# balisujohn/tortoise.cpp

Measured on AMD Instinct MI355X. Metric: audio-seconds/sec end-to-end (AR+diffusion+vocoder), 16 cands x 80 steps, higher is better.
Workload: dtype f16 MFMA inputs / f32 accumulate (diffusion, vocoder convs); f32 weights, f16 KV (AR)

## Files before the change

tortoise.cpp_amd/csrc/api.cpp:

```cpp
#include "common.h"
#include <sched.h>
#include <cctype>
#include <cstddef>
#include <cmath>
#include <algorithm>
#include <chrono>
#include <fstream>
#include <new>

using namespace tts;

hipEvent_t tts::prof_event(tts_ctx *c) {
  if (!c->ev_pool.empty()) { hipEvent_t e = c->ev_pool.back(); c->ev_pool.pop_back(); return e; }
  hipEvent_t e = nullptr;
  (void)hipEventCreate(&e);
  return e;
}

template <class F>
static int guarded(tts_ctx *c, F body) {
  try {
    return body();
  } catch (const std::bad_alloc &) {
    return fail(c, TTS_ERR_LIMIT, "out of host memory");
// ... 139 lines not shown
}

int tts_set_option(tts_ctx *c, const char *key, double value) {
  if (!c || !key) return TTS_ERR_ARG;
  std::string k(key);
  if (k == "gn_eps") c->gn_eps = (float)value;
  else if (k == "ggml_lut") c->ggml_lut = value != 0;
  else if (k.rfind("prof_only:", 0) == 0) {
    if (value != 0) c->prof_filter.push_back(k.substr(10));
    else c->prof_filter.clear();
  }
  else if (k == "device_topk") c->device_topk = value != 0;
  else if (k == "sampler_threads") {
    if (c->sampler_pool) { sampler_pool_free(c->sampler_pool); c->sampler_pool = nullptr; }
    c->sampler_threads = value < 0 ? -1 : (int)value;
  }
  else if (k == "share_uncond") c->share_uncond = value != 0;
  else if (k == "prof_stride") c->prof_stride = value < 1 ? 1 : (int)value;
  else if (k == "diff_graph") c->diff_graph = value != 0;
  else if (k == "dec_f32_mfma") c->dec_f32_mfma = value != 0;
  else if (k == "attn_f32") c->attn_f32 = value != 0;
  else if (k == "attn_proj_f16") c->attn_proj_f16 = value != 0;
  else if (k == "proj_dual_b") c->proj_dual_b = value != 0;
  else if (k == "gemm_wreg") c->gemm_wreg = value == 1 ? tts_ctx::GEMM_WREG_ALL : value == 2 ? 1 : value == 3 ? 2 : value == 4 ? 4 : 0;
  else if (k == "lc_attn_f32") c->lc_attn_f32 = value != 0;
  else if (k == "latency_mode") c->latency_mode = value != 0;
  else if (k == "fp16_check") c->fp16_check = value != 0;
  else if (k == "rng_fast_normal") c->rng_fast_normal = value != 0;
  else if (k == "noise_pipeline") c->noise_pipeline = value != 0;
  else if (k == "load_device_pack") c->load_device_pack = value != 0;
  else if (k == "load_threads") c->load_threads = value < 0 ? 0 : value > 64 ? 64 : (int)value;
  else if (k == "attn_q64") c->attn_q64 = value < 0 ? 0 : value > 2 ? 2 : (int)value;
  else if (k == "hoist_integrator") c->hoist_integrator = value < 0 ? 0 : (int)value;
  else if (k == "attn_f32_drop") c->attn_f32_drop = (int)value & 7;
  else if (k == "ar_weights") {
    if (value != 0 && value != 1 && value != 2) return fail(c, TTS_ERR_ARG, "ar_weights: 0 (f32), 1 (fp16) or 2 (fp8 e4m3)");
    c->ar_weights = (int)value;
  }
  else if (k == "diff_sampler") {
    if (const char *e = diff_control_error(0, value)) return fail(c, TTS_ERR_ARG, "%s", e);
    c->diff_sampler = (int)value;
  }
  else if (k == "ddim_eta") {
    if (const char *e = diff_control_error(1, value)) return fail(c, TTS_ERR_ARG, "%s", e);
    c->ddim_eta = value;
  }
  else if (k == "cond_free_k") {
// ... 712 lines not shown
```

tortoise.cpp_amd/csrc/common.h:

```cpp
#pragma once
#include "../../include/tortoise_mi355x.h"
#include <hip/hip_runtime.h>
#include <cstdarg>
#include <cstdint>
#include <cstdio>
#include <cstring>
#include <functional>
#include <map>
#include <memory>
#include <random>
#include <algorithm>
#include <atomic>
#include <condition_variable>
#include <mutex>
#include <new>
#include <string>
#include <thread>
#include <vector>

namespace tts {

struct HostTensor {
  std::vector<float> data;
  int64_t ne[4] = {1, 1, 1, 1};
// ... 98 lines not shown
  tts::DiffCondEncState *dcond = nullptr;
  tts::HifiganState *hifigan = nullptr;
  tts::AfeState *afe = nullptr;
  tts::Tokenizer *tok = nullptr;
  tts::ArSession *session = nullptr;
  tts::DiffSession *diff_session = nullptr;
  tts::SamplerPool *sampler_pool = nullptr;
  tts::SamplerParams ar_sp;
  int ar_penalty_scope = 0;
  int device_topk = 1;
  int time_mlp_retries = 0;
  int topk_fallbacks = 0;
  int sampler_threads = -1;
  bool share_uncond = true;
  int rng_shard_offset = 0, rng_shard_total = 0;
  std::vector<int32_t> stop_schedule;
  std::vector<int32_t> ar_stopped;
  bool prof_on = false;
  std::vector<std::string> prof_filter;
  int prof_stride = 1;
  int ar_weights = 0;
  int dec_f32_mfma = 0;
  int attn_f32 = 0;
  static constexpr int GEMM_WREG_ALL = 7;
  int gemm_wreg = GEMM_WREG_ALL;
  int proj_dual_b = 1;
  int attn_f32_drop = 0;
  int lc_attn_f32 = 1;
  int attn_proj_f16 = 0;
  int fp16_check = 0;
  int64_t fp16_bad_weights[2] = {0, 0};
  void *fp16_counts = nullptr;
  int rng_fast_normal = 1;
  int noise_pipeline = 1;
  int load_device_pack = 1;
  int load_threads = 0;
  int attn_q64 = 0;
  int hoist_integrator = 1;
  int latency_mode = 0;
  int diff_sampler = 0;
  double ddim_eta = 0;
  float cond_free_k = 2.0f;
  int cond_free = 1;
  double diff_temperature = 1.0;
  int last_diff_rows = -1, last_diff_seqs = 0;
  bool capturing = false;
  int stream_recaptures = 0;
// ... 324 lines not shown
```

tortoise.cpp_amd/csrc/diffusion.hip:

```cpp
#include "common.h"
#include "gemm_f16.h"
#include <algorithm>
#include <chrono>
#include <cmath>

namespace tts {

static constexpr int C = 1024, NHEAD = 16, XTC = 128 ;
static constexpr int LAT_MAX_ROWS = 2048;
static constexpr int HOIST_MAX_ROWS = 16384;

__device__ __forceinline__ float silu_dev(float x, int lut) {
  if (lut == 1) {
    float xr = __half2float(__float2half_rn(x));
    return __half2float(__float2half_rn(xr / (1.0f + expf(-xr))));
  }
  if (lut == 2) return x / (1.0f + expf(-x));
  return x * __builtin_amdgcn_rcpf(1.0f + __builtin_amdgcn_exp2f(x * -1.44269504088896f));
}

__global__ __launch_bounds__(256) void gn_stats_kernel(const float *__restrict__ x, const int *__restrict__ seq_start,
                                                       const int *__restrict__ seq_len, float eps, float2 *__restrict__ stats) {
  __shared__ float sh[8];
  const int grp = blockIdx.x, s = blockIdx.y, T = seq_len[s];
// ... 738 lines not shown
}

__global__ void philox_fill_kernel(float *__restrict__ x, int64_t n, uint64_t seed, uint32_t stream, uint32_t step) {
  int64_t i = (int64_t)blockIdx.x * blockDim.x + threadIdx.x;
  if (i < n) x[i] = philox_normal(seed, stream, step, (uint32_t)i);
}
__global__ void scale_xT_kernel(float *__restrict__ x, int64_t n, float temperature) {
  int64_t i = (int64_t)blockIdx.x * blockDim.x + threadIdx.x;
  if (i < n) x[i] = temperature * x[i];
}

__global__ void rows_to_ct_kernel(const float *__restrict__ net, int row0, int T, int nch, int ld, float *__restrict__ out) {
  int i = blockIdx.x * blockDim.x + threadIdx.x;
  if (i < nch * T) {
    int ch = i / T, t = i - ch * T;
    out[i] = net[(size_t)(row0 + t) * ld + ch];
  }
}

struct AttnDev {
  float *norm_g, *norm_b, *qkv_b, *proj_b, *bias_tab;
  __half *qkv_w, *proj_w;
  __half *qkv_wf;
  __half *proj_w_split;
  float proj_alpha;
};
struct ResDev { float *in_g, *in_b, *in_bias, *emb_w, *emb_b, *out_g, *out_b, *out_bias; __half *in_w, *out_w, *in_wf, *out_wf; };

struct Layout {
  int ns = 0, rows = 0;
  std::vector<int> start, len;
  DevBuf d_row_seq, d_row_t, d_start, d_len, d_chunk_seq;
  int build(tts_ctx *ctx, const std::vector<int> &lens) {
    has_seq_step = false; ss_step_stride = 0; gn_parts.clear();
    ns = (int)lens.size();
    len = lens;
    start.resize(ns);
    int r = 8;
    for (int s = 0; s < ns; s++) { start[s] = r; r = (r + lens[s] + 1 + 7) & ~7; }
    rows = (r + 127) & ~127;
    std::vector<int> rs(rows, -1), rt(rows, 0);
    for (int s = 0; s < ns; s++)
      for (int t = 0; t < lens[s]; t++) { rs[start[s] + t] = s; rt[start[s] + t] = t; }
    TTS_HIP(ctx, d_row_seq.reserve(rows * 4)); TTS_HIP(ctx, d_row_t.reserve(rows * 4));
    TTS_HIP(ctx, d_start.reserve(ns * 4)); TTS_HIP(ctx, d_len.reserve(ns * 4));
    TTS_HIP(ctx, hipMemcpy(d_row_seq.p, rs.data(), rows * 4, hipMemcpyHostToDevice));
// ... 229 lines not shown
  int f32(const std::string &name, int64_t n, float **dst) {
    const HostTensor *t = get(name, n);
    if (!t) return TTS_ERR_FORMAT;
    return put(t->data, dst);
  }
  int conv16(const std::string &name, int cout, int cin, int k, int cout_pad, int cin_pad, __half **dst, __half **dst_frag = nullptr) {
    const HostTensor *t = get(name, (int64_t)cout * cin * k);
    if (!t) return TTS_ERR_FORMAT;
    std::vector<__half> h((size_t)cout_pad * k * cin_pad, __float2half(0.f));
    const float *w = t->data.data();
    for (int co = 0; co < cout; co++)
      for (int ci = 0; ci < cin; ci++)
        for (int tap = 0; tap < k; tap++)
          h[(size_t)co * k * cin_pad + (size_t)tap * cin_pad + ci] = __float2half_rn(w[((size_t)co * cin + ci) * k + tap]);
    if (dst_frag) {
      std::vector<__half> f(h.size());
      for (int n = 0; n < cout_pad; n++)
        for (int tap = 0; tap < k; tap++)
          for (int c = 0; c < cin_pad; c++) f[gemm_wfrag3_index(n, tap, c, cout_pad, cin_pad)] = h[((size_t)n * k + tap) * cin_pad + c];
      if (int r = put(f, dst_frag)) return r;
    }
    return put(h, dst);
  }
  int attn(const std::string &p, AttnDev &a) {
    int r;
    if ((r = f32(p + ".norm.weight", C, &a.norm_g))) return r;
    if ((r = f32(p + ".norm.bias", C, &a.norm_b))) return r;
    if ((r = conv16(p + ".qkv.weight", 3 * C, C, 1, 3 * C, C, &a.qkv_w, &a.qkv_wf))) return r;
    if ((r = f32(p + ".qkv.bias", 3 * C, &a.qkv_b))) return r;
    if ((r = conv16(p + ".proj_out.weight", C, C, 1, C, C, &a.proj_w))) return r;
    {
      const HostTensor *t = get(p + ".proj_out.weight", (int64_t)C * C);
      std::vector<__half> sp((size_t)C * 2 * C);
      float amax = 0.f;
      for (float v : t->data) amax = std::max(amax, std::fabs(v));
      if (!std::isfinite(amax)) { fail(ctx, TTS_ERR_FORMAT, "tensor '%s.proj_out.weight' holds a non-finite value", p.c_str()); return TTS_ERR_FORMAT; }
      int e = 14;
      while (e > -14 && std::ldexp(amax, e) >= 30000.0f) e--;
      const float scale = std::ldexp(1.0f, e);
      a.proj_alpha = 1.0f / scale;
      for (int n = 0; n < C; n++)
        for (int k = 0; k < C; k++) {
          const float w = t->data[(size_t)n * C + k] * scale;
          const __half hi = __float2half_rn(w);
          sp[(size_t)n * 2 * C + k] = hi;
          sp[(size_t)n * 2 * C + C + k] = __float2half_rn(w - __half2float(hi));
        }
      long long bad[2] = {0, 0};
      for (const __half &h : sp) {
        const float v = std::fabs(__half2float(h));
        if (!(v <= 65504.0f)) bad[0]++;
        else if (v > 60000.0f) bad[1]++;
      }
      if (bad[0] | bad[1]) { std::lock_guard<std::mutex> lk(mu); ctx->fp16_bad_weights[0] += bad[0]; ctx->fp16_bad_weights[1] += bad[1]; }
      if ((r = put(sp, &a.proj_w_split))) return r;
    }
    if ((r = f32(p + ".proj_out.bias", C, &a.proj_b))) return r;
    const HostTensor *t = get(p + ".relative_pos_embeddings.relative_attention_bias.weight", 32 * 16);
    if (!t) return TTS_ERR_FORMAT;
    std::vector<float> tab(16 * 128);
    for (int h = 0; h < 16; h++)
      for (int sgn = 0; sgn < 2; sgn++)
        for (int d = 0; d < 64; d++) {
          int bucket = sgn ? rel_bucket(0, d) : rel_bucket(d, 0);
          if (d == 0) bucket = rel_bucket(0, 0);
          tab[h * 128 + sgn * 64 + d] = t->data[(size_t)bucket * 16 + h] * 8.0f;
        }
    return put(tab, &a.bias_tab);
  }
  int res(const std::string &p, ResDev &w) {
    int r;
    if ((r = f32(p + ".in_layers.0.weight", C, &w.in_g))) return r;
    if ((r = f32(p + ".in_layers.0.bias", C, &w.in_b))) return r;
    if ((r = conv16(p + ".in_layers.2.weight", C, C, 1, C, C, &w.in_w, &w.in_wf))) return r;
    if ((r = f32(p + ".in_layers.2.bias", C, &w.in_bias))) return r;
    if ((r = f32(p + ".emb_layers.1.weight", 2 * C * C, &w.emb_w))) return r;
    if ((r = f32(p + ".emb_layers.1.bias", 2 * C, &w.emb_b))) return r;
    if ((r = f32(p + ".out_layers.0.weight", C, &w.out_g))) return r;
// ... 8 lines not shown
int diff_load(tts_ctx *ctx, const char *path) {
  ctx->fp16_bad_weights[0] = ctx->fp16_bad_weights[1] = 0;
  WeightFile wf;
  std::string err;
  int rc = read_weight_file(path, wf, err);
  if (rc != TTS_OK) return fail(ctx, rc, "diffusion_model_load: %s", err.c_str());
  std::unique_ptr<DiffState> st(new DiffState());
  Loader ld{ctx, st.get(), wf, {}};
  while (wf.has("latent_conditioner." + std::to_string(st->n_lc + 1) + ".norm.weight")) st->n_lc++;
  while (wf.has("conditioning_timestep_integrator." + std::to_string(st->n_integ) + ".resblk.in_layers.0.weight")) st->n_integ++;
  while (wf.has("layers." + std::to_string(st->n_main) + ".resblk.in_layers.0.weight")) st->n_main++;
  while (wf.has("layers." + std::to_string(st->n_main + st->n_tail) + ".in_layers.0.weight")) st->n_tail++;
  st->lc_attn.resize(st->n_lc);
  st->integ_res.resize(st->n_integ); st->integ_attn.resize(st->n_integ);
  st->main_res.resize(st->n_main); st->main_attn.resize(st->n_main);
  st->tail_res.resize(st->n_tail);
  std::vector<std::function<int()>> jobs;
  DiffState *S = st.get();
#define J(x) jobs.emplace_back([&ld, S]() -> int { (void)S; return (x); })
  J(ld.f32("diffusion_conditioning_latent", 2 * C, &S->cond_latent));
  J(ld.f32("unconditioned_embedding", C, &S->uncond_emb));
  J(ld.conv16("latent_conditioner.0.weight", C, C, 3, C, C, &S->lc_w));
  J(ld.f32("latent_conditioner.0.bias", C, &S->lc_bias));
  for (int i = 0; i < st->n_lc; i++) jobs.emplace_back([&ld, S, i]() { return ld.attn("latent_conditioner." + std::to_string(i + 1), S->lc_attn[i]); });
  J(ld.f32("code_norm.weight", C, &S->code_g));
  J(ld.f32("code_norm.bias", C, &S->code_b));
  J(ld.f32("time_embed.0.weight", C * C, &S->te0_w)); J(ld.f32("time_embed.0.bias", C, &S->te0_b));
  J(ld.f32("time_embed.2.weight", C * C, &S->te2_w)); J(ld.f32("time_embed.2.bias", C, &S->te2_b));
  for (int i = 0; i < st->n_integ; i++) {
    jobs.emplace_back([&ld, S, i]() { return ld.res("conditioning_timestep_integrator." + std::to_string(i) + ".resblk", S->integ_res[i]); });
    jobs.emplace_back([&ld, S, i]() { return ld.attn("conditioning_timestep_integrator." + std::to_string(i) + ".attn", S->integ_attn[i]); });
  }
  J(ld.conv16("inp_block.weight", C, 100, 3, C, XTC, &S->inp_w));
  J(ld.f32("inp_block.bias", C, &S->inp_bias));
  J(ld.conv16("integrating_conv.weight", C, 2 * C, 1, C, 2 * C, &S->integ_w));
  J(ld.f32("integrating_conv.bias", C, &S->integ_bias));
  for (int i = 0; i < st->n_main; i++) {
    jobs.emplace_back([&ld, S, i]() { return ld.res("layers." + std::to_string(i) + ".resblk", S->main_res[i]); });
    jobs.emplace_back([&ld, S, i]() { return ld.attn("layers." + std::to_string(i) + ".attn", S->main_attn[i]); });
  }
  for (int i = 0; i < st->n_tail; i++) jobs.emplace_back([&ld, S, i]() { return ld.res("layers." + std::to_string(S->n_main + i), S->tail_res[i]); });
  J(ld.f32("out.0.weight", C, &S->outn_g)); J(ld.f32("out.0.bias", C, &S->outn_b));
  J(ld.conv16("out.2.weight", 200, C, 3, 256, C, &S->out_w));
  jobs.emplace_back([&ld, S]() -> int {
    const HostTensor *t = ld.get("out.2.bias", 200);
    if (!t) return TTS_ERR_FORMAT;
    std::vector<float> b(256, 0.f);
    std::copy(t->data.begin(), t->data.end(), b.begin());
    return ld.put(b, &S->out_bias);
  });
#undef J
  if (int r = run_parallel(ctx, (int)jobs.size(), [&](int i) { return jobs[i](); })) return r;
  for (auto &kv : wf.t)
    if (!ld.used.count(kv.first)) return fail(ctx, TTS_ERR_FORMAT, "unknown tensor '%s' in model file", kv.first.c_str());
  TTS_HIP(ctx, hipFuncSetAttribute((const void *)diff_attn_f32_kernel, hipFuncAttributeMaxDynamicSharedMemorySize, ATT32_LDS));
  if (ctx->diff) diff_free(ctx->diff);
  ctx->diff = st.release();
  return TTS_OK;
}

#define CHECK(x) do { int _r = (x); if (_r) return _r; } while (0)

// ... 349 lines not shown
        diff_attn_kernel<2, 2><<<nq * NHEAD * lay.ns, 256, att_lds<2>(), ctx->stream>>>(wk.qk16.as<__half>(), wk.vt16.as<__half>(), wk.rows + 128,
                                                                                    lay.d_start.as<int>(), lay.d_len.as<int>(), w.bias_tab, wk.ATT16(), nq);
    }
    TTS_HIP(ctx, hipGetLastError());
  }
  CHECK(fp16_check(ctx, wk.ATT16(), (size_t)lay.rows * C));
  if (f32 && (ctx->attn_f32_drop & 4)) TTS_HIP(ctx, hipMemsetAsync(wk.att16_lo.p, 0, (size_t)(wk.rows + 2) * C * 2, ctx->stream));
  DBG_SUM("attn out", wk.ATT16(), (size_t)lay.rows * C * 2);
  if (f32) {
    GemmArgs p = gemm_base(lay, wk.ATT16(), C, 3, C, w.proj_w_split, C, w.proj_b);
    p.A[0] = wk.ATT16(); p.A[1] = wk.att16_lo.as<__half>() + C; p.A[2] = wk.ATT16();
    p.row_off[0] = p.row_off[1] = p.row_off[2] = 0;
    p.custom_w = 1; p.ldw_ = 2 * C; p.w_off_[0] = 0; p.w_off_[1] = 0; p.w_off_[2] = C;
    p.mode = st_out ? GEMM_OUT_F32_SCALED_STATS : GEMM_OUT_F32_SCALED; p.alpha = w.proj_alpha; p.outF = X; p.ldo = C; p.resid = X;
    p.st_out = st_out; p.st_stripe_ll = (int)st->gn_stripe_ll; p.chunk_seq = lay.d_chunk_seq.as<int>();
    return gemm(ctx, "diff_gemm", p, lay, 0, C);
  }
  if (!ctx->attn_proj_f16) {
    GemmArgs p = gemm_base(lay, wk.ATT16(), C, 2, C, w.proj_w_split, C, w.proj_b);
    p.custom_w = 1; p.ldw_ = 2 * C; p.w_off_[0] = 0; p.w_off_[1] = C;
    p.mode = st_out ? GEMM_OUT_F32_SCALED_STATS : GEMM_OUT_F32_SCALED; p.alpha = w.proj_alpha; p.outF = X; p.ldo = C; p.resid = X;
    p.st_out = st_out; p.st_stripe_ll = (int)st->gn_stripe_ll; p.chunk_seq = lay.d_chunk_seq.as<int>();
    p.dual_b = ctx->proj_dual_b;
    CHECK(gemm(ctx, "diff_gemm", p, lay, 0, C));
    DBG_SUM("attn proj", X, (size_t)lay.rows * C * 4);
    return TTS_OK;
  }
  GemmArgs p = gemm_base(lay, wk.ATT16(), C, 1, C, w.proj_w, C, w.proj_b);
  p.mode = st_out ? GEMM_OUT_F32_STATS : GEMM_OUT_F32; p.outF = X; p.ldo = C; p.resid = X;
  p.st_out = st_out; p.st_stripe_ll = (int)st->gn_stripe_ll; p.chunk_seq = lay.d_chunk_seq.as<int>();
  CHECK(gemm(ctx, "diff_gemm", p, lay));
  DBG_SUM("attn proj", X, (size_t)lay.rows * C * 4);
  return TTS_OK;
}

static int res_block(tts_ctx *ctx, DiffState *st, const Layout &lay, Work &wk, float *X, const ResDev &w, const float *ss,
                     const float *Xin = nullptr, const float *Hpre = nullptr, const long long *st_hpre = nullptr) {
  const float *xin = Xin ? Xin : X;
  const bool lat = st->lat && (Hpre ? st_hpre != nullptr : wk.st_x != nullptr);
  const long long *st_h = st_hpre;
  if (!Hpre) {
    long long *slot = lat ? st->new_stats_slot() : nullptr;
    CHECK(res_in_layers(ctx, st, lay, wk, xin, w, wk.H(), lat ? wk.st_x : nullptr, slot));
    Hpre = wk.H();
    st_h = slot;
  }
// ... 832 lines not shown
```

tortoise.cpp_amd/csrc/gemm_f16.h:

```cpp
#pragma once
#include <hip/hip_fp16.h>
#include <hip/hip_runtime.h>
#include <algorithm>
#include <cmath>
#include <cstdlib>
#include <type_traits>

namespace tts {

typedef _Float16 half8 __attribute__((ext_vector_type(8)));
typedef float floatx4 __attribute__((ext_vector_type(4)));

enum { GEMM_OUT_F32 = 0, GEMM_OUT_F16 = 1, GEMM_OUT_QKV = 2, GEMM_OUT_QKV_SPLIT = 3, GEMM_OUT_F32_SCALED = 4, GEMM_OUT_F32_STATS = 5, GEMM_OUT_F32_SCALED_STATS = 6 };
constexpr bool gemm_mode_qkv(int mode) { return mode == GEMM_OUT_QKV || mode == GEMM_OUT_QKV_SPLIT; }
constexpr bool gemm_mode_f32(int mode) { return mode == GEMM_OUT_F32 || mode == GEMM_OUT_F32_SCALED || mode == GEMM_OUT_F32_STATS || mode == GEMM_OUT_F32_SCALED_STATS; }
constexpr bool gemm_mode_scaled(int mode) { return mode == GEMM_OUT_F32_SCALED || mode == GEMM_OUT_F32_SCALED_STATS; }
constexpr bool gemm_mode_stats(int mode) { return mode == GEMM_OUT_F32_STATS || mode == GEMM_OUT_F32_SCALED_STATS; }

struct GemmArgs {
  const __half *A[3];
  int row_off[3];
  int nseg, kseg;
  int lda;
  const __half *W;
  int ldw_, w_off_[3], custom_w;
  const __half *Wf;
  int wreg;
  int M, N;
  const float *bias;
  const int *row_seq;
  float *outF; int ldo; const float *resid;
  __half *outH; int ldh;
  __half *outVt; int ldvt;
  __half *outH2, *outVt2;
  float alpha;
  long long *st_out;
  int st_stripe_ll;
  const int *chunk_seq;
  int dual_b;
  int mode;
  int th, cn;
  int ku;
};


__device__ __forceinline__ int lds_swz(int row) { return ((row >> 1) & 3) << 1; }
__device__ __forceinline__ int lds_off(int row, int chunk) { return row * 128 + ((chunk ^ lds_swz(row)) << 4); }

typedef const void __attribute__((address_space(1))) *gptr_t;
// ... 460 lines not shown
#pragma unroll
            for (int r = 0; r < 4; r++) v[r] = gd[r] ? 0.f : acc[i][j][r] + bv[j];
            const size_t o = (size_t)(h * 64 + (w0 - 128) + j * 16 + fr) * g.ldvt + rbase;
            *(uint2 *)(g.outVt + o) = pack_half4(v[0], v[1], v[2], v[3]);
            if (MODE == GEMM_OUT_QKV_SPLIT) *(uint2 *)(g.outVt2 + o) = pack_half4(split_lo(v[0]), split_lo(v[1]), split_lo(v[2]), split_lo(v[3]));
          }
        }
      }
      return;
    }
  }
  const int col0 = c0 + fq * 4;
  float4 b4[2];
  int sq[MI];
#pragma unroll
  for (int j = 0; j < 2; j++) b4[j] = *(const float4 *)(bp + col0 + j * 16);
#pragma unroll
  for (int i = 0; i < MI; i++) sq[i] = sp[m0 + min(i, nblk - 1) * 16 + fr];
#pragma unroll
  for (int j = 0; j < 2; j++) b4[j] = hb ? b4[j] : make_float4(0.f, 0.f, 0.f, 0.f);
#pragma unroll
  for (int i = 0; i < MI; i++) sq[i] = hs ? sq[i] : 0;
  auto finish = [&](int i, int j) {
    float4 v = make_float4(acc[i][j][0] + b4[j].x, acc[i][j][1] + b4[j].y, acc[i][j][2] + b4[j].z, acc[i][j][3] + b4[j].w);
    if (sq[i] < 0) v = make_float4(0.f, 0.f, 0.f, 0.f);
    return v;
  };
  if (MODE == GEMM_OUT_F32) {
#pragma unroll
    for (int i = 0; i < MI; i++) {
      if (i < nblk) {
        float *op = g.outF + (size_t)(m0 + i * 16 + fr) * g.ldo + col0;
#pragma unroll
        for (int j = 0; j < 2; j++) *(float4 *)(op + j * 16) = finish(i, j);
      }
    }
  } else {
    const int h = c0 / 192, w0 = c0 - h * 192;
#pragma unroll
    for (int i = 0; i < MI; i++) {
      if (i < nblk) {
        __half *op = g.outH + (size_t)(m0 + i * 16 + fr) * g.ldh + h * 128 + w0 + fq * 4;
#pragma unroll
        for (int j = 0; j < 2; j++) {
          const float4 v = finish(i, j);
          *(uint2 *)(op + j * 16) = pack_half4(v.x, v.y, v.z, v.w);
          if (MODE == GEMM_OUT_QKV_SPLIT)
            *(uint2 *)(g.outH2 + (op - g.outH) + j * 16) = pack_half4(split_lo(v.x), split_lo(v.y), split_lo(v.z), split_lo(v.w));
        }
      }
    }
// ... 335 lines not shown
  issue_slab(0, 0);
  issue_w(0, 0, std::integral_constant<int, 0>{});
  for (int kc = 0; kc < nchunks; kc += 2) {
    chunk(kc, std::integral_constant<int, 0>{});
    if (kc + 1 < nchunks) chunk(kc + 1, std::integral_constant<int, 1>{});
  }
  wreg_wait<0>(w[0][0][0], w[0][0][1], w[0][1][0], w[0][1][1]);
  wreg_wait<0>(w[1][0][0], w[1][0][1], w[1][1][0], w[1][1][1]);
  gemm_epilogue_conv3_wreg<MI, RESID>(g, acc, m0, n0, nblk, wave, fr, fq);
}

template <bool RESID>
static __global__ __launch_bounds__(256, 4) void gemm_f16_conv3_wreg_kernel(GemmArgs g) {
  const int tid = threadIdx.x, lane = tid & 63, wave = __builtin_amdgcn_readfirstlane(tid >> 6);
  int m0, n0, nblk;
  if (!gemm_vh_tile(g, m0, n0, nblk)) return;
  if (nblk > 4) gemm_conv3_wreg_body<8, RESID>(g, m0, n0, nblk, lane, wave);
  else gemm_conv3_wreg_body<4, RESID>(g, m0, n0, nblk, lane, wave);
}
static inline bool gemm_takes_conv3_wreg(const GemmArgs &g, int th) {
  return g.wreg > 0 && g.Wf && gemm_is_conv3(g) && th == 8 && g.mode == GEMM_OUT_F32;
}

static inline int gemm_auto_th(int M, int N) {
  const int maxb = ((M >> 4) + 7) / 8 + 1, NT = N >> 7;
  int th = 2;
  while (th < 8 && 8 * ((maxb + th - 1) / th) * NT > 1024) th *= 2;
  return th;
}

enum { GEMM_KERNEL_VH = 0, GEMM_KERNEL_DUALB = 1, GEMM_KERNEL_CONV3 = 2, GEMM_KERNEL_WREG = 3, GEMM_KERNEL_CONV3_WREG = 4 };
struct GemmPlan {
  hipError_t err;
  int kernel;
  int th, ku, cn;
  int grid, lds;
};
static inline GemmPlan gemm_plan(const GemmArgs &g) {
  GemmPlan p = {};
  const int NT = g.N >> 7, ktot = g.nseg * g.kseg, nb = g.M >> 4;
  p.err = hipSuccess;
  if (gemm_mode_scaled(g.mode)) {
    int e;
    if (!(g.alpha != 0.f) || std::fabs(std::frexp(g.alpha, &e)) != 0.5f) p.err = hipErrorInvalidValue;
  }
  if (gemm_mode_stats(g.mode) && (!g.st_out || !g.chunk_seq || g.st_stripe_ll <= 0)) p.err = hipErrorInvalidValue;
  if (g.dual_b && !(gemm_mode_scaled(g.mode) && g.nseg == 2 && g.custom_w && g.A[0] == g.A[1] && g.row_off[0] == g.row_off[1])) p.err = hipErrorInvalidValue;
  int ku = (g.ku == 2 || g.ku == 4) && (g.kseg % (64 * g.ku)) == 0 ? g.ku : 1;
  p.cn = NT;
  if (NT > 8)
    for (p.cn = NT; p.cn > 1; p.cn--)
      if (NT % p.cn == 0 && (size_t)p.cn * 128 * ktot * 2 <= (size_t)2560 * 1024) break;
  const int maxb = (nb + 7) / 8 + 1;
  p.th = g.th > 0 ? g.th : gemm_auto_th(g.M, g.N);
  if (g.th <= 0 && g.ku == 0 && NT <= 8 && 8 * ((maxb + 3) / 4) * NT <= 256 && (g.kseg % 256) == 0) {
    p.th = 4;
    if (!gemm_is_conv3(g)) ku = g.dual_b ? 2 : 4;
  }
  int mt_max = 0;
  for (int x = 0; x < 8; x++) {
    const int b0 = (int)((long long)nb * x >> 3), b1 = (int)((long long)nb * (x + 1) >> 3);
    mt_max = std::max(mt_max, (b1 - b0 + p.th - 1) / p.th);
  }
  p.grid = 8 * mt_max * NT;
  if (gemm_takes_wreg(g, p.th, ku)) { p.kernel = GEMM_KERNEL_WREG; p.ku = 1; p.lds = GEMM_WREG_LDS; }
  else if (gemm_takes_conv3_wreg(g, p.th)) { p.kernel = GEMM_KERNEL_CONV3_WREG; p.ku = 1; p.lds = CONV3_WREG_LDS; }
  else if (gemm_is_conv3(g)) { p.kernel = GEMM_KERNEL_CONV3; p.ku = 1; p.lds = CONV3_VH_LDS; }
  else if (g.dual_b) { p.kernel = GEMM_KERNEL_DUALB; p.ku = ku == 2 ? 2 : 1; p.lds = p.ku * GEMM_DUALB_LDS; }
  else { p.kernel = GEMM_KERNEL_VH; p.ku = ku; p.lds = ku * GEMM_VH_LDS; }
  return p;
}

static_assert(GEMM_DUALB_LDS <= 48 * 1024 && GEMM_VH_LDS <= 48 * 1024 && GEMM_WREG_LDS <= 48 * 1024 && CONV3_WREG_LDS <= 48 * 1024 && CONV3_VH_LDS > 48 * 1024, "which launches raise their dynamic LDS limit");
template <void (*KERN)(GemmArgs)> static inline void gemm_launch(const GemmPlan &p, const GemmArgs &g, hipStream_t s) {
  if (p.lds > 48 * 1024) {
    static bool raised = false;
    if (!raised) { (void)hipFuncSetAttribute((const void *)KERN, hipFuncAttributeMaxDynamicSharedMemorySize, p.lds); raised = true; }
  }
  KERN<<<p.grid, 256, p.lds, s>>>(g);
}
template <int KU> static inline void gemm_launch_vh(const GemmPlan &p, const GemmArgs &g, hipStream_t s) {
  constexpr int WGS = KU == 1 ? 4 : KU == 2 ? 2 : 1;
  switch (g.mode) {
    case GEMM_OUT_F32: return gemm_launch<gemm_f16_vh_kernel<GEMM_OUT_F32, WGS, KU>>(p, g, s);
    case GEMM_OUT_F16: return gemm_launch<gemm_f16_vh_kernel<GEMM_OUT_F16, WGS, KU>>(p, g, s);
    case GEMM_OUT_QKV: return gemm_launch<gemm_f16_vh_kernel<GEMM_OUT_QKV, WGS, KU>>(p, g, s);
    case GEMM_OUT_QKV_SPLIT: return gemm_launch<gemm_f16_vh_kernel<GEMM_OUT_QKV_SPLIT, WGS, KU>>(p, g, s);
    case GEMM_OUT_F32_SCALED: return gemm_launch<gemm_f16_vh_kernel<GEMM_OUT_F32_SCALED, WGS, KU>>(p, g, s);
    case GEMM_OUT_F32_STATS: return gemm_launch<gemm_f16_vh_kernel<GEMM_OUT_F32_STATS, WGS, KU>>(p, g, s);
    default: return gemm_launch<gemm_f16_vh_kernel<GEMM_OUT_F32_SCALED_STATS, WGS, KU>>(p, g, s);
  }
}
template <int KU> static inline void gemm_launch_dualb(const GemmPlan &p, const GemmArgs &g, hipStream_t s) {
  if (g.mode == GEMM_OUT_F32_SCALED) gemm_launch<gemm_f16_vh_dualb_kernel<GEMM_OUT_F32_SCALED, KU>>(p, g, s);
  else gemm_launch<gemm_f16_vh_dualb_kernel<GEMM_OUT_F32_SCALED_STATS, KU>>(p, g, s);
}
// ... 1 lines not shown
  if (g.mode == GEMM_OUT_F32) gemm_launch<gemm_f16_conv3_vh_kernel<GEMM_OUT_F32>>(p, g, s);
  else if (g.mode == GEMM_OUT_F32_STATS) gemm_launch<gemm_f16_conv3_vh_kernel<GEMM_OUT_F32_STATS>>(p, g, s);
  else gemm_launch<gemm_f16_conv3_vh_kernel<GEMM_OUT_F16>>(p, g, s);
}
static inline void gemm_launch_conv3_wreg(const GemmPlan &p, const GemmArgs &g, hipStream_t s) {
  if (g.resid) gemm_launch<gemm_f16_conv3_wreg_kernel<true>>(p, g, s);
  else gemm_launch<gemm_f16_conv3_wreg_kernel<false>>(p, g, s);
}
static inline void gemm_launch_wreg(const GemmPlan &p, const GemmArgs &g, hipStream_t s) {
  if (g.mode == GEMM_OUT_F32) gemm_launch<gemm_f16_wreg_kernel<GEMM_OUT_F32>>(p, g, s);
  else if (g.mode == GEMM_OUT_QKV) gemm_launch<gemm_f16_wreg_kernel<GEMM_OUT_QKV>>(p, g, s);
  else gemm_launch<gemm_f16_wreg_kernel<GEMM_OUT_QKV_SPLIT>>(p, g, s);
}

static inline hipError_t launch_gemm_f16(const GemmArgs &g, hipStream_t s) {
  const GemmPlan p = gemm_plan(g);
  if (p.err != hipSuccess) return p.err;
  GemmArgs gg = g;
  gg.th = p.th;
  gg.cn = p.cn;
  if (p.kernel == GEMM_KERNEL_WREG) gemm_launch_wreg(p, gg, s);
  else if (p.kernel == GEMM_KERNEL_CONV3_WREG) gemm_launch_conv3_wreg(p, gg, s);
  else if (p.kernel == GEMM_KERNEL_CONV3) gemm_launch_conv3(p, gg, s);
  else if (p.kernel == GEMM_KERNEL_DUALB) p.ku == 2 ? gemm_launch_dualb<2>(p, gg, s) : gemm_launch_dualb<1>(p, gg, s);
  else p.ku == 4 ? gemm_launch_vh<4>(p, gg, s) : p.ku == 2 ? gemm_launch_vh<2>(p, gg, s) : gemm_launch_vh<1>(p, gg, s);
  return hipGetLastError();
}

}
```

Baseline: 137.5.

## Add register-resident weight dual-B GEMM kernel for diffusion attention projection

Adds a new dual-B GEMM kernel for the attention output projection in the diffusion model. It loads pre-packed fragment-ordered weights straight into registers, while A tiles stream through LDS with double buffering. The load path builds the packed weight image for integrator and main-layer attention blocks, and the planner routes the scaled dual-B case to the new kernel when th==8. The aim is to cut LDS traffic and weight staging for the projection GEMM, at the cost of extra weight memory and a new, complex hand-scheduled kernel. The wreg epilogue gains alpha scaling for the scaled mode, and a test harness is added.

Measured after the change: 138.7, median of 6. About the same (+0.9%).

```diff
diff --git a/tortoise.cpp_amd/csrc/api.cpp b/tortoise.cpp_amd/csrc/api.cpp
--- a/tortoise.cpp_amd/csrc/api.cpp
+++ b/tortoise.cpp_amd/csrc/api.cpp
@@ -185,7 +185,7 @@
   else if (k == "attn_f32") c->attn_f32 = value != 0;
   else if (k == "attn_proj_f16") c->attn_proj_f16 = value != 0;
   else if (k == "proj_dual_b") c->proj_dual_b = value != 0;
-  else if (k == "gemm_wreg") c->gemm_wreg = value == 1 ? tts_ctx::GEMM_WREG_ALL : value == 2 ? 1 : value == 3 ? 2 : value == 4 ? 4 : 0;
+  else if (k == "gemm_wreg") c->gemm_wreg = value == 1 ? tts_ctx::GEMM_WREG_ALL : value == 2 ? 1 : value == 3 ? 2 : value == 4 ? 4 : value == 5 ? 8 : 0;
   else if (k == "lc_attn_f32") c->lc_attn_f32 = value != 0;
   else if (k == "latency_mode") c->latency_mode = value != 0;
   else if (k == "fp16_check") c->fp16_check = value != 0;
diff --git a/tortoise.cpp_amd/csrc/common.h b/tortoise.cpp_amd/csrc/common.h
--- a/tortoise.cpp_amd/csrc/common.h
+++ b/tortoise.cpp_amd/csrc/common.h
@@ -144,7 +144,7 @@
   int ar_weights = 0;
   int dec_f32_mfma = 0;
   int attn_f32 = 0;
-  static constexpr int GEMM_WREG_ALL = 7;
+  static constexpr int GEMM_WREG_ALL = 15;
   int gemm_wreg = GEMM_WREG_ALL;
   int proj_dual_b = 1;
   int attn_f32_drop = 0;
diff --git a/tortoise.cpp_amd/csrc/diffusion.hip b/tortoise.cpp_amd/csrc/diffusion.hip
--- a/tortoise.cpp_amd/csrc/diffusion.hip
+++ b/tortoise.cpp_amd/csrc/diffusion.hip
@@ -784,6 +784,7 @@
   float *norm_g, *norm_b, *qkv_b, *proj_b, *bias_tab;
   __half *qkv_w, *proj_w;
   __half *qkv_wf;
+  __half *proj_wf2 = nullptr;
   __half *proj_w_split;
   float proj_alpha;
 };
@@ -1059,7 +1060,7 @@
     }
     return put(h, dst);
   }
-  int attn(const std::string &p, AttnDev &a) {
+  int attn(const std::string &p, AttnDev &a, bool split_image) {
     int r;
     if ((r = f32(p + ".norm.weight", C, &a.norm_g))) return r;
     if ((r = f32(p + ".norm.bias", C, &a.norm_b))) return r;
@@ -1091,6 +1092,15 @@
       }
       if (bad[0] | bad[1]) { std::lock_guard<std::mutex> lk(mu); ctx->fp16_bad_weights[0] += bad[0]; ctx->fp16_bad_weights[1] += bad[1]; }
       if ((r = put(sp, &a.proj_w_split))) return r;
+      if (split_image) {
+        std::vector<__half> f(sp.size());
+        for (int n = 0; n < C; n++)
+          for (int k = 0; k < C; k++) {
+            f[gemm_wfrag2_index(n, 1, k, C)] = sp[(size_t)n * 2 * C + k];
+            f[gemm_wfrag2_index(n, 0, k, C)] = sp[(size_t)n * 2 * C + C + k];
+          }
+        if ((r = put(f, &a.proj_wf2))) return r;
+      }
     }
     if ((r = f32(p + ".proj_out.bias", C, &a.proj_b))) return r;
     const HostTensor *t = get(p + ".relative_pos_embeddings.relative_attention_bias.weight", 32 * 16);
@@ -1145,14 +1155,14 @@
   J(ld.f32("unconditioned_embedding", C, &S->uncond_emb));
   J(ld.conv16("latent_conditioner.0.weight", C, C, 3, C, C, &S->lc_w));
   J(ld.f32("latent_conditioner.0.bias", C, &S->lc_bias));
-  for (int i = 0; i < st->n_lc; i++) jobs.emplace_back([&ld, S, i]() { return ld.attn("latent_conditioner." + std::to_string(i + 1), S->lc_attn[i]); });
+  for (int i = 0; i < st->n_lc; i++) jobs.emplace_back([&ld, S, i]() { return ld.attn("latent_conditioner." + std::to_string(i + 1), S->lc_attn[i], false); });
   J(ld.f32("code_norm.weight", C, &S->code_g));
   J(ld.f32("code_norm.bias", C, &S->code_b));
   J(ld.f32("time_embed.0.weight", C * C, &S->te0_w)); J(ld.f32("time_embed.0.bias", C, &S->te0_b));
   J(ld.f32("time_embed.2.weight", C * C, &S->te2_w)); J(ld.f32("time_embed.2.bias", C, &S->te2_b));
   for (int i = 0; i < st->n_integ; i++) {
     jobs.emplace_back([&ld, S, i]() { return ld.res("conditioning_timestep_integrator." + std::to_string(i) + ".resblk", S->integ_res[i]); });
-    jobs.emplace_back([&ld, S, i]() { return ld.attn("conditioning_timestep_integrator." + std::to_string(i) + ".attn", S->integ_attn[i]); });
+    jobs.emplace_back([&ld, S, i]() { return ld.attn("conditioning_timestep_integrator." + std::to_string(i) + ".attn", S->integ_attn[i], true); });
   }
   J(ld.conv16("inp_block.weight", C, 100, 3, C, XTC, &S->inp_w));
   J(ld.f32("inp_block.bias", C, &S->inp_bias));
@@ -1160,7 +1170,7 @@
   J(ld.f32("integrating_conv.bias", C, &S->integ_bias));
   for (int i = 0; i < st->n_main; i++) {
     jobs.emplace_back([&ld, S, i]() { return ld.res("layers." + std::to_string(i) + ".resblk", S->main_res[i]); });
-    jobs.emplace_back([&ld, S, i]() { return ld.attn("layers." + std::to_string(i) + ".attn", S->main_attn[i]); });
+    jobs.emplace_back([&ld, S, i]() { return ld.attn("layers." + std::to_string(i) + ".attn", S->main_attn[i], true); });
   }
   for (int i = 0; i < st->n_tail; i++) jobs.emplace_back([&ld, S, i]() { return ld.res("layers." + std::to_string(S->n_main + i), S->tail_res[i]); });
   J(ld.f32("out.0.weight", C, &S->outn_g)); J(ld.f32("out.0.bias", C, &S->outn_b));
@@ -1556,6 +1566,7 @@
     p.mode = st_out ? GEMM_OUT_F32_SCALED_STATS : GEMM_OUT_F32_SCALED; p.alpha = w.proj_alpha; p.outF = X; p.ldo = C; p.resid = X;
     p.st_out = st_out; p.st_stripe_ll = (int)st->gn_stripe_ll; p.chunk_seq = lay.d_chunk_seq.as<int>();
     p.dual_b = ctx->proj_dual_b;
+    p.Wf2 = w.proj_wf2; p.wreg = gemm_wreg_class(ctx, 8);
     CHECK(gemm(ctx, "diff_gemm", p, lay, 0, C));
     DBG_SUM("attn proj", X, (size_t)lay.rows * C * 4);
     return TTS_OK;
diff --git a/tortoise.cpp_amd/csrc/gemm_f16.h b/tortoise.cpp_amd/csrc/gemm_f16.h
--- a/tortoise.cpp_amd/csrc/gemm_f16.h
+++ b/tortoise.cpp_amd/csrc/gemm_f16.h
@@ -25,6 +25,7 @@
   const __half *W;
   int ldw_, w_off_[3], custom_w;
   const __half *Wf;
+  const __half *Wf2;
   int wreg;
   int M, N;
   const float *bias;
@@ -531,11 +532,12 @@
 #pragma unroll
   for (int i = 0; i < MI; i++) sq[i] = hs ? sq[i] : 0;
   auto finish = [&](int i, int j) {
+    if (gemm_mode_scaled(MODE)) acc[i][j] *= g.alpha;
     float4 v = make_float4(acc[i][j][0] + b4[j].x, acc[i][j][1] + b4[j].y, acc[i][j][2] + b4[j].z, acc[i][j][3] + b4[j].w);
     if (sq[i] < 0) v = make_float4(0.f, 0.f, 0.f, 0.f);
     return v;
   };
-  if (MODE == GEMM_OUT_F32) {
+  if (MODE == GEMM_OUT_F32 || MODE == GEMM_OUT_F32_SCALED) {
 #pragma unroll
     for (int i = 0; i < MI; i++) {
       if (i < nblk) {
@@ -917,6 +919,116 @@
   return g.wreg > 0 && g.Wf && gemm_is_conv3(g) && th == 8 && g.mode == GEMM_OUT_F32;
 }
 
+static inline size_t gemm_wfrag2_index(int n, int half, int k, int K) {
+  return (((((size_t)(n >> 4) * (K >> 5) + (k >> 5)) * 2 + half) * 64 + ((k >> 3) & 3) * 16 + (n & 15)) << 3) + (k & 7);
+}
+static constexpr int GEMM_DUALB_WREG_LDS = 2 * 16384;
+
+template <int MI>
+__device__ __forceinline__ void gemm_dualb_wreg_body(const GemmArgs &g, int m0, int n0, int nblk, int lane, int wave) {
+  extern __shared__ __attribute__((aligned(16))) char smem_dyn[];
+  char *smem = smem_dyn;
+  constexpr int MODE = GEMM_OUT_F32_SCALED;
+  constexpr int NPA = MI / 2;
+  const int T = g.kseg >> 6, KS = g.kseg >> 5;
+  const int fr = lane & 15, fq = lane >> 4;
+  unsigned aoff[NPA];
+#pragma unroll
+  for (int i = 0; i < NPA; i++) aoff[i] = (unsigned)(gemm_dma_off(wave + 4 * i, lane, 0, nblk * 16 - 1, g.lda) * 2);
+  const char *aseg = (const char *)(g.A[0] + (ptrdiff_t)(g.row_off[0] + m0) * g.lda);
+  const __half *wp0 = g.Wf2 + (size_t)((n0 >> 4) + wave * 2) * KS * 1024, *wp1 = wp0 + (size_t)KS * 1024;
+  const unsigned wlane = lane * 16;
+  const bool resid_first = g.resid != nullptr;
+  floatx4 acc[MI][2];
+  gemm_acc_start<MODE, MI, 2>(g, acc, resid_first, n0 + wave * 32, fq, [&](int i) { return m0 + min(i, nblk - 1) * 16 + fr; });
+  int fbase[2];
+#pragma unroll
+  for (int ks = 0; ks < 2; ks++) {
+    fbase[ks] = lds_off(fr, ks * 4 + fq);
+    asm volatile("" : "+v"(fbase[ks]));
+  }
+  half8 w[2][2][2];
+  auto issue_w = [&](int s, auto set_c) {
+    constexpr int U = decltype(set_c)::value;
+    const __half *q0 = wp0 + (size_t)min(s, KS - 1) * 1024, *q1 = wp1 + (size_t)min(s, KS - 1) * 1024;
+    wreg_load<0>(w[U][0][0], q0, wlane);
+    wreg_load<0>(w[U][0][1], q1, wlane);
+    wreg_load<1024>(w[U][1][0], q0, wlane);
+    wreg_load<1024>(w[U][1][1], q1, wlane);
+  };
+  auto issue_a = [&](int t, int slot) {
+    const char *ab = aseg + (min(t, T - 1) << 7);
+    asm volatile("" : "+s"(ab));
+#pragma unroll
+    for (int i = 0; i < NPA; i++) {
+      unsigned o = aoff[i];
+      asm volatile("" : "+v"(o));
+      __builtin_amdgcn_global_load_lds((gptr_t)(ab + o), (lptr_t)(smem + slot * 16384 + (wave + 4 * i) * 1024), 16, 0, 0);
+    }
+  };
+  auto step = [&](int t, auto par_c, auto ks_c) {
+    constexpr int PAR = decltype(par_c)::value, U = decltype(ks_c)::value;
+    if (U == 0) {
+      wreg_wait<0>(w[0][0][0], w[0][0][1], w[0][1][0], w[0][1][1]);
+      asm volatile("s_waitcnt lgkmcnt(0)" ::: "memory");
+      __builtin_amdgcn_s_barrier();
+    } else {
+      wreg_wait<NPA>(w[1][0][0], w[1][0][1], w[1][1][0], w[1][1][1]);
+    }
+    issue_w(2 * t + U + 1, std::integral_constant<int, U ^ 1>{});
+    if (U == 0) issue_a(t + 1, PAR ^ 1);
+    const char *sa = smem + PAR * 16384 + fbase[U];
+    constexpr int AHEAD = 2;
+    half8 af[AHEAD + 1];
+    auto frag = [&](int i) { return *(const half8 *)(sa + i * 2048); };
+#pragma unroll
+    for (int x = 0; x < AHEAD; x++) af[x] = frag(x);
+#pragma unroll
+    for (int i = 0; i < MI; i++) {
+      if (i + AHEAD < MI) af[(i + AHEAD) % (AHEAD + 1)] = frag(i + AHEAD);
+      const half8 a = af[i % (AHEAD + 1)];
+#pragma unroll
+      for (int j = 0; j < 2; j++) acc[i][j] = __builtin_amdgcn_mfma_f32_16x16x32_f16(w[U][0][j], a, acc[i][j], 0, 0, 0);
+#pragma unroll
+      for (int j = 0; j < 2; j++) acc[i][j] = __builtin_amdgcn_mfma_f32_16x16x32_f16(w[U][1][j], a, acc[i][j], 0, 0, 0);
+    }
+    __builtin_amdgcn_sched_group_barrier(0x100, AHEAD, 0);
+#pragma unroll
+    for (int i = 0; i < MI; i++) {
+      if (i + AHEAD < MI) __builtin_amdgcn_sched_group_barrier(0x100, 1, 0);
+      __builtin_amdgcn_sched_group_barrier(0x008, 4, 0);
+    }
+  };
+  auto tile = [&](int t, auto par_c) {
+    step(t, par_c, std::integral_constant<int, 0>{});
+    step(t, par_c, std::integral_constant<int, 1>{});
+  };
+  issue_a(0, 0);
+  issue_w(0, std::integral_constant<int, 0>{});
+#pragma unroll
+  for (int i = 0; i < MI; i++)
+#pragma unroll
+    for (int j = 0; j < 2; j++) asm volatile("" : "+v"(acc[i][j]));
+  for (int t = 0; t < T; t += 2) {
+    tile(t, std::integral_constant<int, 0>{});
+    if (t + 1 < T) tile(t + 1, std::integral_constant<int, 1>{});
+  }
+  wreg_wait<0>(w[0][0][0], w[0][0][1], w[0][1][0], w[0][1][1]);
+  wreg_wait<0>(w[1][0][0], w[1][0][1], w[1][1][0], w[1][1][1]);
+  gemm_epilogue_wreg<MODE, MI, false>(g, acc, m0, n0, nblk, wave, fr, fq);
+}
+
+static __global__ __launch_bounds__(256, 4) void gemm_f16_dualb_wreg_kernel(GemmArgs g) {
+  const int tid = threadIdx.x, lane = tid & 63, wave = __builtin_amdgcn_readfirstlane(tid >> 6);
+  int m0, n0, nblk;
+  if (!gemm_vh_tile(g, m0, n0, nblk)) return;
+  if (nblk > 4) gemm_dualb_wreg_body<8>(g, m0, n0, nblk, lane, wave);
+  else gemm_dualb_wreg_body<4>(g, m0, n0, nblk, lane, wave);
+}
+static inline bool gemm_takes_dualb_wreg(const GemmArgs &g, int th, int ku) {
+  return g.dual_b && g.wreg > 0 && g.Wf2 && th == 8 && ku == 1 && g.mode == GEMM_OUT_F32_SCALED && (g.kseg % 64) == 0 && g.kseg >= 128;
+}
+
 static inline int gemm_auto_th(int M, int N) {
   const int maxb = ((M >> 4) + 7) / 8 + 1, NT = N >> 7;
   int th = 2;
@@ -924,7 +1036,7 @@
   return th;
 }
 
-enum { GEMM_KERNEL_VH = 0, GEMM_KERNEL_DUALB = 1, GEMM_KERNEL_CONV3 = 2, GEMM_KERNEL_WREG = 3, GEMM_KERNEL_CONV3_WREG = 4 };
+enum { GEMM_KERNEL_VH = 0, GEMM_KERNEL_DUALB = 1, GEMM_KERNEL_CONV3 = 2, GEMM_KERNEL_WREG = 3, GEMM_KERNEL_CONV3_WREG = 4, GEMM_KERNEL_DUALB_WREG = 5 };
 struct GemmPlan {
   hipError_t err;
   int kernel;
@@ -961,12 +1073,13 @@
   if (gemm_takes_wreg(g, p.th, ku)) { p.kernel = GEMM_KERNEL_WREG; p.ku = 1; p.lds = GEMM_WREG_LDS; }
   else if (gemm_takes_conv3_wreg(g, p.th)) { p.kernel = GEMM_KERNEL_CONV3_WREG; p.ku = 1; p.lds = CONV3_WREG_LDS; }
   else if (gemm_is_conv3(g)) { p.kernel = GEMM_KERNEL_CONV3; p.ku = 1; p.lds = CONV3_VH_LDS; }
+  else if (gemm_takes_dualb_wreg(g, p.th, ku)) { p.kernel = GEMM_KERNEL_DUALB_WREG; p.ku = 1; p.lds = GEMM_DUALB_WREG_LDS; }
   else if (g.dual_b) { p.kernel = GEMM_KERNEL_DUALB; p.ku = ku == 2 ? 2 : 1; p.lds = p.ku * GEMM_DUALB_LDS; }
   else { p.kernel = GEMM_KERNEL_VH; p.ku = ku; p.lds = ku * GEMM_VH_LDS; }
   return p;
 }
 
-static_assert(GEMM_DUALB_LDS <= 48 * 1024 && GEMM_VH_LDS <= 48 * 1024 && GEMM_WREG_LDS <= 48 * 1024 && CONV3_WREG_LDS <= 48 * 1024 && CONV3_VH_LDS > 48 * 1024, "which launches raise their dynamic LDS limit");
+static_assert(GEMM_DUALB_LDS <= 48 * 1024 && GEMM_VH_LDS <= 48 * 1024 && GEMM_WREG_LDS <= 48 * 1024 && CONV3_WREG_LDS <= 48 * 1024 && GEMM_DUALB_WREG_LDS <= 48 * 1024 && CONV3_VH_LDS > 48 * 1024, "which launches raise their dynamic LDS limit");
 template <void (*KERN)(GemmArgs)> static inline void gemm_launch(const GemmPlan &p, const GemmArgs &g, hipStream_t s) {
   if (p.lds > 48 * 1024) {
     static bool raised = false;
@@ -1014,6 +1127,7 @@
   if (p.kernel == GEMM_KERNEL_WREG) gemm_launch_wreg(p, gg, s);
   else if (p.kernel == GEMM_KERNEL_CONV3_WREG) gemm_launch_conv3_wreg(p, gg, s);
   else if (p.kernel == GEMM_KERNEL_CONV3) gemm_launch_conv3(p, gg, s);
+  else if (p.kernel == GEMM_KERNEL_DUALB_WREG) gemm_launch<gemm_f16_dualb_wreg_kernel>(p, gg, s);
   else if (p.kernel == GEMM_KERNEL_DUALB) p.ku == 2 ? gemm_launch_dualb<2>(p, gg, s) : gemm_launch_dualb<1>(p, gg, s);
   else p.ku == 4 ? gemm_launch_vh<4>(p, gg, s) : p.ku == 2 ? gemm_launch_vh<2>(p, gg, s) : gemm_launch_vh<1>(p, gg, s);
   return hipGetLastError();
diff --git a/tortoise.cpp_amd/testlib/gemm_dualb_harness.hip b/tortoise.cpp_amd/testlib/gemm_dualb_harness.hip
--- /dev/null
+++ b/tortoise.cpp_amd/testlib/gemm_dualb_harness.hip
@@ -0,0 +1,162 @@
+#include "../csrc/gemm_f16.h"
+
+#include <cstdint>
+#include <cstdio>
+#include <cstring>
+#include <vector>
+
+using namespace tts;
+
+extern "C" {
+
+enum { TTS_DUALB_TEST_MARGIN = 4096, TTS_DUALB_TEST_SENTINEL = 0xCB };
+
+struct tts_gemm_case {
+  int M, N, nseg, kseg;
+  int row_off[3], a_sel[3];
+  int mode, th, ku, wreg, dual_b, custom_w, ldw, w_off[3];
+  float alpha;
+  int has_bias, has_resid, resid_aliases_out, has_row_seq, has_chunk_seq, has_st;
+  int lda, ldo, ldh, ldvt, nseq, st_stripe_ll, launches;
+  const uint16_t *A0, *A1, *W;
+  const float *bias, *resid;
+  const int *row_seq, *chunk_seq;
+  float *outF;
+  uint16_t *outH, *outH2, *outVt, *outVt2;
+  long long *st;
+};
+
+int tts_dualb_test_margin(void) { return TTS_DUALB_TEST_MARGIN; }
+long long tts_dualb_test_wfrag2_index(int n, int half, int k, int K) { return (long long)gemm_wfrag2_index(n, half, k, K); }
+int tts_dualb_test_pack(const uint16_t *W, int N, int K, int ldw, int off_hi, int off_lo, uint16_t *img) {
+  if (!W || !img || N < 16 || (N & 15) || K < 32 || (K & 31) || off_hi < 0 || off_lo < 0 || off_hi + K > ldw || off_lo + K > ldw) return (int)hipErrorInvalidValue;
+  for (int n = 0; n < N; n++)
+    for (int k = 0; k < K; k++) {
+      img[gemm_wfrag2_index(n, 1, k, K)] = W[(size_t)n * ldw + off_hi + k];
+      img[gemm_wfrag2_index(n, 0, k, K)] = W[(size_t)n * ldw + off_lo + k];
+    }
+  return 0;
+}
+
+}
+
+namespace {
+
+char g_last[160] = "none";
+
+GemmArgs host_args(const tts_gemm_case &c) {
+  static const __half dummy[2] = {};
+  GemmArgs g;
+  memset(&g, 0, sizeof g);
+  for (int s = 0; s < 3; s++) {
+    g.A[s] = dummy;
+    g.row_off[s] = c.row_off[s];
+    g.w_off_[s] = c.w_off[s];
+  }
+  g.nseg = c.nseg; g.kseg = c.kseg; g.lda = c.lda; g.custom_w = c.custom_w; g.ldw_ = c.ldw;
+  g.wreg = c.wreg; g.M = c.M; g.N = c.N; g.ldo = c.ldo; g.alpha = c.alpha;
+  g.st_stripe_ll = c.st_stripe_ll; g.dual_b = c.dual_b; g.mode = c.mode; g.th = c.th; g.ku = c.ku;
+  return g;
+}
+
+void describe(const GemmArgs &g, char *buf, int cap) {
+  static const char *const names[] = {"vh", "dualb", "conv3", "wreg", "conv3w", "dualbw"};
+  const GemmPlan p = gemm_plan(g);
+  snprintf(buf, cap, "%s mode=%d th=%d ku=%d cn=%d grid=%d lds=%d err=%d", names[p.kernel], g.mode, p.th, p.ku, p.cn, p.grid, p.lds, (int)p.err);
+}
+
+struct Dev {
+  char *p = nullptr;
+  size_t bytes = 0;
+  ~Dev() { if (p) (void)hipFree(p); }
+  hipError_t alloc(size_t payload, int fill) {
+    bytes = payload;
+    hipError_t e = hipMalloc((void **)&p, payload + 2 * TTS_DUALB_TEST_MARGIN);
+    if (e != hipSuccess) { p = nullptr; return e; }
+    return hipMemset(p, fill, payload + 2 * TTS_DUALB_TEST_MARGIN);
+  }
+  char *data() const { return p + TTS_DUALB_TEST_MARGIN; }
+  hipError_t put(const void *h) { return hipMemcpy(data(), h, bytes, hipMemcpyHostToDevice); }
+  hipError_t get_all(void *h) const { return hipMemcpy(h, p, bytes + 2 * TTS_DUALB_TEST_MARGIN, hipMemcpyDeviceToHost); }
+};
+
+bool valid(const tts_gemm_case &c, bool run) {
+  if (c.M < 16 || c.M > 131072 || (c.M & 15) || c.N < 128 || c.N > 4096 || (c.N & 127)) return false;
+  if (c.kseg < 64 || c.kseg > 4096 || (c.kseg & 63)) return false;
+  if (c.nseg != 2 || !c.dual_b || !c.custom_w || c.a_sel[0] || c.a_sel[1] || c.row_off[0] != 0 || c.row_off[1] != 0) return false;
+  if (c.mode != GEMM_OUT_F32_SCALED && c.mode != GEMM_OUT_F32_SCALED_STATS) return false;
+  if (c.th < 0 || c.th > 8 || !(c.ku == 0 || c.ku == 1 || c.ku == 2 || c.ku == 4) || c.launches < 1 || c.launches > 2) return false;
+  if (c.lda < c.kseg || c.lda < 64 || (c.lda & 7) || !c.A0 || !c.W) return false;
+  if (c.ldw < 2 * c.kseg || (c.ldw & 7)) return false;
+  for (int s = 0; s < 2; s++)
+    if (c.w_off[s] < 0 || (c.w_off[s] & 7) || c.w_off[s] + c.kseg > c.ldw) return false;
+  if (c.has_bias && !c.bias) return false;
+  if (c.has_row_seq && !c.row_seq) return false;
+  if (c.has_resid && !c.resid) return false;
+  if (c.resid_aliases_out && !c.has_resid) return false;
+  if ((run && !c.outF) || c.ldo < c.N || (c.ldo & 3)) return false;
+  if (c.mode == GEMM_OUT_F32_SCALED_STATS) {
+    if (run) return false;
+  }
+  return true;
+}
+
+}
+
+extern "C" {
+
+int tts_dualb_test_plan(const tts_gemm_case *c, int image, char *buf, int cap) {
+  if (!c || !buf || cap <= 0 || !valid(*c, false)) return (int)hipErrorInvalidValue;
+  GemmArgs g = host_args(*c);
+  static const __half placeholder[1] = {};
+  static long long st_placeholder[1] = {};
+  static const int cs_placeholder[1] = {};
+  if (image) g.Wf2 = placeholder;
+  if (c->mode == GEMM_OUT_F32_SCALED_STATS) { g.st_out = st_placeholder; g.chunk_seq = cs_placeholder; if (g.st_stripe_ll <= 0) g.st_stripe_ll = 128; }
+  describe(g, buf, cap);
+  return 0;
+}
+
+int tts_dualb_test_last_kernel(char *buf, int cap) {
+  if (!buf || cap <= 0) return (int)hipErrorInvalidValue;
+  snprintf(buf, cap, "%s", g_last);
+  return 0;
+}
+
+#define HT(x) do { hipError_t e_ = (x); if (e_ != hipSuccess) return (int)e_; } while (0)
+
+int tts_dualb_test_run(const tts_gemm_case *cp, int image) {
+  if (!cp || !valid(*cp, true)) return (int)hipErrorInvalidValue;
+  const tts_gemm_case &c = *cp;
+  const size_t a_bytes = (size_t)(c.M + 2) * c.lda * 2, w_bytes = (size_t)c.N * c.ldw * 2, i_bytes = (size_t)c.N * 2 * c.kseg * 2;
+  const size_t f_bytes = (size_t)c.M * c.ldo * 4;
+  Dev a0, w, wf2, bias, resid, rseq, outF;
+  GemmArgs g = host_args(c);
+  HT(a0.alloc(a_bytes, 0)); HT(a0.put(c.A0));
+  HT(w.alloc(w_bytes, 0)); HT(w.put(c.W));
+  for (int s = 0; s < 3; s++) g.A[s] = (const __half *)a0.data() + c.lda;
+  g.W = (const __half *)w.data();
+  if (image) {
+    std::vector<uint16_t> img((size_t)c.N * 2 * c.kseg);
+    if (tts_dualb_test_pack(c.W, c.N, c.kseg, c.ldw, c.w_off[0], c.w_off[1], img.data())) return (int)hipErrorInvalidValue;
+    HT(wf2.alloc(i_bytes, 0)); HT(wf2.put(img.data()));
+    g.Wf2 = (const __half *)wf2.data();
+  }
+  if (c.has_bias) { HT(bias.alloc((size_t)c.N * 4, 0)); HT(bias.put(c.bias)); g.bias = (const float *)bias.data(); }
+  if (c.has_row_seq) { HT(rseq.alloc((size_t)c.M * 4, 0xFF)); HT(rseq.put(c.row_seq)); g.row_seq = (const int *)rseq.data(); }
+  HT(outF.alloc(f_bytes, TTS_DUALB_TEST_SENTINEL));
+  g.outF = (float *)outF.data();
+  if (c.has_resid && c.resid_aliases_out) { HT(outF.put(c.resid)); g.resid = g.outF; }
+  else if (c.has_resid) { HT(resid.alloc(f_bytes, 0)); HT(resid.put(c.resid)); g.resid = (const float *)resid.data(); }
+  describe(g, g_last, sizeof g_last);
+  hipStream_t s;
+  HT(hipStreamCreateWithFlags(&s, hipStreamNonBlocking));
+  hipError_t e = hipDeviceSynchronize();
+  for (int l = 0; l < c.launches && e == hipSuccess; l++) e = launch_gemm_f16(g, s);
+  const hipError_t es = hipStreamSynchronize(s);
+  (void)hipStreamDestroy(s);
+  HT(outF.get_all(c.outF));
+  return (int)(e != hipSuccess ? e : es);
+}
+
+}
```
